# gopi-erabati/SRFDet3D

Hardware: AMD Instinct MI355X
Metric: frames/sec, srfdet_voxel_nusc_LC synthetic 30k-pt sweeps (higher is better)
Workload: dtype f32

## Files before the change

srfdet3d_amd/csrc/wino43.hip:

```cpp
#include "common.hpp"
#include <algorithm>

typedef float w43_f32x16 __attribute__((ext_vector_type(16)));
typedef float w43_f32x4 __attribute__((ext_vector_type(4)));
typedef float w43_v2 __attribute__((ext_vector_type(2)));

#define W43_TB 32
#define W43_PIECE 1024
#define W43_X1_BYTES (36 * 8 * 64 * 4)
#define W43_X_BYTES (36 * 16 * 64 * 4)

struct W43Args {
    const float *x;
    float *y;
    float *V;
    const float *U;
    const float *scale, *shift;
    long long x_ld, y_ld;
    int N, H, W, Cout;
    int tilesX, tilesY;
    long long ntiles;
    int ntb, nchunk, ncb, relu;
    int tb0, n0;
};

__global__ __launch_bounds__(256) void srf_wino43_pack_k(const float *__restrict__ Wt, int Cout, int Cin, int nchunk, float *__restrict__ P,
                                                        long long total)
{
    const long long t = (long long)blockIdx.x * 256 + threadIdx.x;
    if (t >= total) return;
    const int kk = (int)(t & 3), co = (int)((t >> 2) & 31), q = (int)((t >> 7) & 1), h = (int)((t >> 8) & 1);
    long long rest = t >> 9;
    const int f = (int)(rest % 36);
    rest /= 36;
    const int chunk = (int)(rest % nchunk), cb = (int)(rest / nchunk);
    const int cog = cb * 64 + h * 32 + co, ci = chunk * 8 + q * 4 + kk;
    float r = 0.f;
    if (cog < Cout) {
        const double G[6][3] = {{0.25, 0.0, 0.0},
                                {-1.0 / 6, -1.0 / 6, -1.0 / 6},
                                {-1.0 / 6, 1.0 / 6, -1.0 / 6},
                                {1.0 / 24, 1.0 / 12, 1.0 / 6},
                                {1.0 / 24, -1.0 / 12, 1.0 / 6},
                                {0.0, 0.0, 1.0}};
        const float *g = Wt + ((size_t)cog * Cin + ci) * 9;
        const int fr = f / 6, fs = f - fr * 6;
        double s = 0.0;
#pragma unroll
        for (int a = 0; a < 3; ++a)
#pragma unroll
            for (int b = 0; b < 3; ++b) s += G[fr][a] * (double)g[a * 3 + b] * G[fs][b];
        r = (float)s;
    }
    P[t] = r;
}

__device__ __forceinline__ float4 w43_fma4(float s, float4 a, float4 b)
{
    return make_float4(__fmaf_rn(s, a.x, b.x), __fmaf_rn(s, a.y, b.y), __fmaf_rn(s, a.z, b.z), __fmaf_rn(s, a.w, b.w));
}
__device__ __forceinline__ float4 w43_add4(float4 a, float4 b) { return make_float4(a.x + b.x, a.y + b.y, a.z + b.z, a.w + b.w); }
__device__ __forceinline__ float4 w43_sub4(float4 a, float4 b) { return make_float4(a.x - b.x, a.y - b.y, a.z - b.z, a.w - b.w); }

#define W43_BT(X0, X1, X2, X3, X4, X5, V0, V1, V2, V3, V4, V5)   \
    do {                                                         \
        const float4 a_ = w43_fma4(-4.f, X2, X4);                \
        const float4 b_ = w43_fma4(-4.f, X1, X3);                \
        const float4 c_ = w43_sub4(X4, X2);                      \
        const float4 e_ = w43_sub4(X3, X1);                      \
        const float4 v0_ = w43_fma4(4.f, X0, w43_fma4(-5.f, X2, X4)); \
        const float4 v5_ = w43_fma4(4.f, X1, w43_fma4(-5.f, X3, X5)); \
        V0 = v0_;                                                \
        V1 = w43_add4(a_, b_);                                   \
        V2 = w43_sub4(a_, b_);                                   \
        V3 = w43_fma4(2.f, e_, c_);                              \
        V4 = w43_fma4(-2.f, e_, c_);                             \
        V5 = v5_;                                                \
    } while (0)

__global__ __launch_bounds__(256) void srf_wino43_xform_k(W43Args a)
{
    const int tid = threadIdx.x, lane = tid & 63, wave = __builtin_amdgcn_readfirstlane(tid >> 6);
    const int cgroups = (a.nchunk + 3) >> 2;
    const int tbl = blockIdx.x / cgroups, cg = blockIdx.x - tbl * cgroups;
    const int qd = lane & 7, t = wave * 8 + (lane >> 3);
    const int c = cg * 4 + (qd >> 1), q = qd & 1;
    const bool c_ok = c < a.nchunk;
    const int g = (a.tb0 + tbl) * W43_TB + t;
    const int per_img = a.tilesX * a.tilesY;
    const bool live = g < (int)a.ntiles;
    const int n = live ? g / per_img : a.n0;
    const int rem = live ? g - n * per_img : 0;
    const int ty = rem / a.tilesX, tx = rem - ty * a.tilesX;
    const long long img_b = (long long)a.H * a.W * a.x_ld * 4;
    const long long left_b = (long long)(a.N - a.n0) * img_b;
    __amdgpu_buffer_rsrc_t xr = __builtin_amdgcn_make_buffer_rsrc(const_cast<float *>(a.x), 0,
                                                                 (int)(unsigned)(left_b < 0xFFFFFFF0ll ? left_b : 0xFFFFFFF0ll), 0x00020000);
    const int y0 = 4 * ty - 1, x0 = 4 * tx - 1;
    const unsigned px_b = (unsigned)(a.x_ld * 4);
    const unsigned chan_b = (unsigned)((c * 8 + q * 4) * 4) + (unsigned)(n - a.n0) * (unsigned)img_b;
    const bool share = (lane < 56) && live && (g + 1 < (int)a.ntiles) && (tx + 1 < a.tilesX);
    float4 d[6][6];
#pragma unroll
    for (int py = 0; py < 6; ++py) {
        const int y = y0 + py;
        const bool yok = live && c_ok && y >= 0 && y < a.H;
        const unsigned row_b = (unsigned)(y * a.W) * px_b + chan_b;
#pragma unroll
        for (int px = 0; px < 6; ++px) {
            const int x = x0 + px;
            const bool ok = yok && x >= 0 && x < a.W && !(px >= 4 && share);
            const unsigned off = ok ? row_b + (unsigned)x * px_b : 0xFFFFFFF8u;
            auto v_ = __builtin_amdgcn_raw_buffer_load_b128(xr, (int)off, 0, 0);
            d[py][px] = *reinterpret_cast<float4 *>(&v_);
        }
    }
#pragma unroll
    for (int py = 0; py < 6; ++py)
#pragma unroll
        for (int px = 4; px < 6; ++px) {
            const float4 nb = d[py][px - 4];
            const float sx = __shfl_down(nb.x, 8), sy = __shfl_down(nb.y, 8), sz = __shfl_down(nb.z, 8), sw = __shfl_down(nb.w, 8);
            if (share) d[py][px] = make_float4(sx, sy, sz, sw);
        }
    if (!c_ok) return;
#pragma unroll
    for (int px = 0; px < 6; ++px)
        W43_BT(d[0][px], d[1][px], d[2][px], d[3][px], d[4][px], d[5][px], d[0][px], d[1][px], d[2][px], d[3][px], d[4][px], d[5][px]);
    float4 *vp = reinterpret_cast<float4 *>(a.V) + ((size_t)tbl * a.nchunk + c) * (36 * 64) + q * 32 + t;
#pragma unroll
    for (int r = 0; r < 6; ++r) {
        float4 v0, v1, v2, v3, v4, v5;
        W43_BT(d[r][0], d[r][1], d[r][2], d[r][3], d[r][4], d[r][5], v0, v1, v2, v3, v4, v5);
        vp[(r * 6 + 0) * 64] = v0;
        vp[(r * 6 + 1) * 64] = v1;
        vp[(r * 6 + 2) * 64] = v2;
        vp[(r * 6 + 3) * 64] = v3;
        vp[(r * 6 + 4) * 64] = v4;
        vp[(r * 6 + 5) * 64] = v5;
    }
}

__device__ __forceinline__ w43_v2 w43_pk_add(w43_v2 a, w43_v2 b)
{
    w43_v2 r;
    asm("v_pk_add_f32 %0, %1, %2" : "=v"(r) : "v"(a), "v"(b));
    return r;
}
__device__ __forceinline__ w43_v2 w43_pk_sub(w43_v2 a, w43_v2 b)
{
    w43_v2 r;
    asm("v_pk_add_f32 %0, %1, %2 neg_lo:[0,1] neg_hi:[0,1]" : "=v"(r) : "v"(a), "v"(b));
    return r;
}
__device__ __forceinline__ w43_v2 w43_pk_fma(w43_v2 s, w43_v2 a, w43_v2 b)
{
    w43_v2 r;
    asm("v_pk_fma_f32 %0, %1, %2, %3" : "=v"(r) : "v"(s), "v"(a), "v"(b));
    return r;
}
#define W43_AT(M0, M1, M2, M3, M4, M5, Z0, Z1, Z2, Z3)           \
    do {                                                         \
        const w43_v2 s1_ = w43_pk_add(M1, M2), d1_ = w43_pk_sub(M1, M2); \
        const w43_v2 s2_ = w43_pk_add(M3, M4), d2_ = w43_pk_sub(M3, M4); \
        Z0 = w43_pk_add(w43_pk_add(M0, s1_), s2_);               \
        Z1 = w43_pk_fma(k2_, d2_, d1_);                          \
        Z2 = w43_pk_fma(k4_, s2_, s1_);                          \
        Z3 = w43_pk_add(w43_pk_fma(k8_, d2_, d1_), M5);          \
    } while (0)

#define W43_MFMA(ACC, A, B) ACC = __builtin_amdgcn_mfma_f32_32x32x2f32(A, B, ACC, 0, 0, 0)

template <int NB>
__device__ __forceinline__ void srf_wino43_mm_body(const W43Args &a, const int tb, const int hb)
{
    extern __shared__ __attribute__((aligned(16))) float s_x[];
    const int tid = threadIdx.x, lane = tid & 63, wave = __builtin_amdgcn_readfirstlane(tid >> 6);
    const int li = lane & 31, lh = lane >> 5;
    const int cb = hb >> 1, h0 = hb & 1;
    const int nchunk = a.nchunk;
    __amdgpu_buffer_rsrc_t vr = __builtin_amdgcn_make_buffer_rsrc(
        const_cast<float *>(a.V) + (size_t)(tb - a.tb0) * nchunk * (36 * 256), 0, (int)((long long)nchunk * 36 * W43_PIECE), 0x00020000);
    __amdgpu_buffer_rsrc_t ur = __builtin_amdgcn_make_buffer_rsrc(
        const_cast<float *>(a.U) + (size_t)cb * nchunk * (36 * 2 * 256), 0, (int)((long long)nchunk * 36 * 2 * W43_PIECE), 0x00020000);
    const int voff = lane * 16;
    const int fbase = wave * 9;

    w43_f32x16 acc[9][NB];
    w43_f32x4 fa[9], fb[9][NB];
#define W43_LOAD(J, C)                                                                                                   \
    do {                                                                                                                 \
        const int sa_ = ((C) * 36 + fbase + (J)) * W43_PIECE;                                                            \
        auto va_ = __builtin_amdgcn_raw_buffer_load_b128(vr, voff, sa_, 0);                                              \
        fa[J] = *reinterpret_cast<w43_f32x4 *>(&va_);                                                                    \
        _Pragma("unroll") for (int h_ = 0; h_ < NB; ++h_) {                                                              \
            const int sb_ = (((C) * 36 + fbase + (J)) * 2 + (NB == 2 ? h_ : h0)) * W43_PIECE;                            \
            auto vb_ = __builtin_amdgcn_raw_buffer_load_b128(ur, voff, sb_, 0);                                          \
            fb[J][h_] = *reinterpret_cast<w43_f32x4 *>(&vb_);                                                            \
        }                                                                                                                \
    } while (0)
#define W43_MFMA_V(ACC, A, B) asm volatile("v_mfma_f32_32x32x2_f32 %0, %1, %2, %0" : "+v"(ACC) : "v"(A), "v"(B))
#define W43_MFMA_V0(ACC, A, B) asm volatile("v_mfma_f32_32x32x2_f32 %0, %1, %2, 0" : "=&v"(ACC) : "v"(A), "v"(B))
#define W43_GROUP(J, FIRST)                                                                                              \
    do {                                                                                                                 \
        _Pragma("unroll") for (int s_ = 0; s_ < 4; ++s_)                                                                 \
            _Pragma("unroll") for (int h_ = 0; h_ < NB; ++h_) {                                                          \
                if (NB == 2 && (J) == 8) {                                                                               \
                    if ((FIRST) && s_ == 0) W43_MFMA_V0(acc[J][h_], fa[J][s_], fb[J][h_][s_]);                           \
                    else W43_MFMA_V(acc[J][h_], fa[J][s_], fb[J][h_][s_]);                                               \
                } else if ((FIRST) && s_ == 0) {                                                                         \
                    const w43_f32x16 z_ = {0.f, 0.f, 0.f, 0.f, 0.f, 0.f, 0.f, 0.f, 0.f, 0.f, 0.f, 0.f, 0.f, 0.f, 0.f, 0.f}; \
                    acc[J][h_] = __builtin_amdgcn_mfma_f32_32x32x2f32(fa[J][s_], fb[J][h_][s_], z_, 0, 0, 0);            \
                } else                                                                                                   \
                    W43_MFMA(acc[J][h_], fa[J][s_], fb[J][h_][s_]);                                                      \
            }                                                                                                            \
    } while (0)

#pragma unroll
    for (int j = 0; j < 9; ++j) W43_LOAD(j, 0);
    if (nchunk > 1) {
#pragma unroll
        for (int j = 0; j < 9; ++j) {
            W43_GROUP(j, 1);
            W43_LOAD(j, 1);
            __builtin_amdgcn_sched_barrier(0);
        }
        for (int c = 1; c < nchunk - 1; ++c) {
#pragma unroll
            for (int j = 0; j < 9; ++j) {
                W43_GROUP(j, 0);
                W43_LOAD(j, c + 1);
                __builtin_amdgcn_sched_barrier(0);
            }
        }
#pragma unroll
        for (int j = 0; j < 9; ++j) W43_GROUP(j, 0);
    } else {
#pragma unroll
        for (int j = 0; j < 9; ++j) W43_GROUP(j, 1);
    }

    asm volatile("s_nop 15\n\ts_nop 15" ::: "memory");
    const w43_v2 k2_ = {2.f, 2.f}, k4_ = {4.f, 4.f}, k8_ = {8.f, 8.f};
    float *X = s_x;
    const int per_img = a.tilesX * a.tilesY;
    const unsigned ypx_b = (unsigned)(a.y_ld * 4), yrow_b = (unsigned)a.W * ypx_b;
    const long long yleft_b = (long long)(a.N - a.n0) * a.H * a.W * a.y_ld * 4;
    __amdgpu_buffer_rsrc_t yr = __builtin_amdgcn_make_buffer_rsrc(a.y, 0, (int)(unsigned)(yleft_b < 0xFFFFFFF0ll ? yleft_b : 0xFFFFFFF0ll), 0x00020000);
    if constexpr (NB == 1) {
        const w43_v2 *X2 = reinterpret_cast<const w43_v2 *>(s_x);
        const int er = tid >> 5, ep = tid & 31;
        const int co = cb * 64 + h0 * 32 + 2 * (ep & 15);
        const bool co_ok = co < a.Cout;
        w43_v2 sc = {1.f, 1.f}, sh = {0.f, 0.f};
        if (co_ok && a.scale) sc = *reinterpret_cast<const w43_v2 *>(a.scale + co);
        if (co_ok && a.shift) sh = *reinterpret_cast<const w43_v2 *>(a.shift + co);
#pragma unroll
        for (int ph = 0; ph < 2; ++ph) {
            const int r = ph * 8 + er;
            const int et = (r & 3) + 8 * (r >> 2) + 4 * (ep >> 4);
            const int eg = tb * W43_TB + et;
            const bool elive = eg < (int)a.ntiles;
            const int en = elive ? eg / per_img : a.n0;
            const int erem = elive ? eg - en * per_img : 0;
            const int ety = erem / a.tilesX, etx = erem - ety * a.tilesX;
            const int rows_ok = elive ? min(4, a.H - 4 * ety) : 0, cols_ok = min(4, a.W - 4 * etx);
            const unsigned ebase = (unsigned)(en - a.n0) * ((unsigned)a.H * yrow_b) + (unsigned)(4 * ety) * yrow_b + (unsigned)(4 * etx) * ypx_b;
            __syncthreads();
#pragma unroll
            for (int j = 0; j < 9; ++j)
#pragma unroll
                for (int rr = 0; rr < 8; ++rr) X[((fbase + j) * 8 + rr) * 64 + lane] = acc[j][0][ph * 8 + rr];
            __syncthreads();
            w43_v2 z[4][6];
#pragma unroll
            for (int s = 0; s < 6; ++s) {
                const w43_v2 m0 = X2[((0 * 6 + s) * 8 + er) * 32 + ep], m1 = X2[((1 * 6 + s) * 8 + er) * 32 + ep],
                             m2 = X2[((2 * 6 + s) * 8 + er) * 32 + ep], m3 = X2[((3 * 6 + s) * 8 + er) * 32 + ep],
                             m4 = X2[((4 * 6 + s) * 8 + er) * 32 + ep], m5 = X2[((5 * 6 + s) * 8 + er) * 32 + ep];
                W43_AT(m0, m1, m2, m3, m4, m5, z[0][s], z[1][s], z[2][s], z[3][s]);
            }
#pragma unroll
            for (int i = 0; i < 4; ++i) {
                w43_v2 o[4];
                W43_AT(z[i][0], z[i][1], z[i][2], z[i][3], z[i][4], z[i][5], o[0], o[1], o[2], o[3]);
#pragma unroll
                for (int jx = 0; jx < 4; ++jx) {
                    w43_v2 v = w43_pk_fma(o[jx], sc, sh);
                    if (a.relu) {
                        v[0] = fmaxf(v[0], 0.f);
                        v[1] = fmaxf(v[1], 0.f);
                    }
                    const bool ok = co_ok && i < rows_ok && jx < cols_ok;
                    const unsigned off = ok ? ebase + (unsigned)i * yrow_b + (unsigned)jx * ypx_b + (unsigned)co * 4u : 0xFFFFFFF8u;
                    typedef unsigned w43_u2 __attribute__((ext_vector_type(2)));
                    const w43_u2 bits = {__float_as_uint(v[0]), __float_as_uint(v[1])};
                    __builtin_amdgcn_raw_buffer_store_b64(bits, yr, (int)off, 0, 0);
                }
            }
        }
    } else {
    const float4 *X4 = reinterpret_cast<const float4 *>(s_x);
    const int er = tid >> 4, eq = tid & 15;
    const int et = (er & 3) + 8 * (er >> 2) + 4 * (eq >> 3);
    const int co4 = (eq & 7) * 4;
    const int eg = tb * W43_TB + et;
    const bool elive = eg < (int)a.ntiles;
    const int en = elive ? eg / per_img : a.n0;
    const int erem = elive ? eg - en * per_img : 0;
    const int ety = erem / a.tilesX, etx = erem - ety * a.tilesX;
    const int rows_ok = elive ? min(4, a.H - 4 * ety) : 0, cols_ok = min(4, a.W - 4 * etx);
    const unsigned ebase = (unsigned)(en - a.n0) * ((unsigned)a.H * yrow_b) + (unsigned)(4 * ety) * yrow_b + (unsigned)(4 * etx) * ypx_b;
#pragma unroll
    for (int p = 0; p < NB; ++p) {
        __syncthreads();
#pragma unroll
        for (int j = 0; j < 9; ++j)
#pragma unroll
            for (int r = 0; r < 16; ++r) X[((fbase + j) * 16 + r) * 64 + lane] = acc[j][p][r];
        __syncthreads();
        const int co = cb * 64 + (NB == 2 ? p : h0) * 32 + co4;
        const bool co_ok = co < a.Cout;
        float4 sc = make_float4(1.f, 1.f, 1.f, 1.f), sh = make_float4(0.f, 0.f, 0.f, 0.f);
        if (co_ok && a.scale) sc = *reinterpret_cast<const float4 *>(a.scale + co);
        if (co_ok && a.shift) sh = *reinterpret_cast<const float4 *>(a.shift + co);
        const w43_v2 scl = {sc.x, sc.y}, sch = {sc.z, sc.w}, shl = {sh.x, sh.y}, shh = {sh.z, sh.w};
        w43_v2 zl[4][6], zh[4][6];
#pragma unroll
        for (int s = 0; s < 6; ++s) {
            float4 m[6];
#pragma unroll
            for (int r = 0; r < 6; ++r) m[r] = X4[((r * 6 + s) * 16 + er) * 16 + eq];
            const w43_v2 l0 = {m[0].x, m[0].y}, l1 = {m[1].x, m[1].y}, l2 = {m[2].x, m[2].y}, l3 = {m[3].x, m[3].y}, l4 = {m[4].x, m[4].y},
                         l5 = {m[5].x, m[5].y};
            const w43_v2 h0_ = {m[0].z, m[0].w}, h1 = {m[1].z, m[1].w}, h2 = {m[2].z, m[2].w}, h3 = {m[3].z, m[3].w}, h4 = {m[4].z, m[4].w},
                         h5 = {m[5].z, m[5].w};
            W43_AT(l0, l1, l2, l3, l4, l5, zl[0][s], zl[1][s], zl[2][s], zl[3][s]);
            W43_AT(h0_, h1, h2, h3, h4, h5, zh[0][s], zh[1][s], zh[2][s], zh[3][s]);
        }
#pragma unroll
        for (int i = 0; i < 4; ++i) {
            w43_v2 ol[4], oh[4];
            W43_AT(zl[i][0], zl[i][1], zl[i][2], zl[i][3], zl[i][4], zl[i][5], ol[0], ol[1], ol[2], ol[3]);
            W43_AT(zh[i][0], zh[i][1], zh[i][2], zh[i][3], zh[i][4], zh[i][5], oh[0], oh[1], oh[2], oh[3]);
#pragma unroll
            for (int jx = 0; jx < 4; ++jx) {
                w43_v2 vl = w43_pk_fma(ol[jx], scl, shl), vh = w43_pk_fma(oh[jx], sch, shh);
                if (a.relu) {
                    vl[0] = fmaxf(vl[0], 0.f);
                    vl[1] = fmaxf(vl[1], 0.f);
                    vh[0] = fmaxf(vh[0], 0.f);
                    vh[1] = fmaxf(vh[1], 0.f);
                }
                const bool ok = co_ok && i < rows_ok && jx < cols_ok;
                const unsigned off = ok ? ebase + (unsigned)i * yrow_b + (unsigned)jx * ypx_b + (unsigned)co * 4u : 0xFFFFFFF8u;
                typedef unsigned w43_u4 __attribute__((ext_vector_type(4)));
                const w43_u4 bits = {__float_as_uint(vl[0]), __float_as_uint(vl[1]), __float_as_uint(vh[0]), __float_as_uint(vh[1])};
                __builtin_amdgcn_raw_buffer_store_b128(bits, yr, (int)off, 0, 0);
            }
        }
    }
    }
}

template <int NB>
__global__ __launch_bounds__(256, NB == 1 ? 2 : 1) void srf_wino43_mm_k(W43Args a, int nitems_cb)
{
    const int xcd = blockIdx.x & 7, jq = blockIdx.x >> 3;
    const int cbi = jq % nitems_cb;
    const int tb = a.tb0 + (jq / nitems_cb) * 8 + xcd;
    if (tb >= a.ntb) return;
    srf_wino43_mm_body<NB>(a, tb, NB == 2 ? 2 * cbi : cbi);
}

extern "C" size_t srf_wino43_packed_weight_bytes(int Cout, int Cin)
{
    if (Cout <= 0 || Cin <= 0 || (Cin & 7)) return 0;
    return (size_t)srf_ceil_div(Cout, 64) * (Cin / 8) * 36 * 2 * W43_PIECE;
}

extern "C" int srf_wino43_pack_weights(const float *W, int Cout, int Cin, float *packed, srf_stream_t stream)
{
    if (Cout <= 0 || Cin <= 0 || !W || !packed) return SRF_EINVAL;
    if (Cin & 7) return SRF_EUNSUPPORTED;
    const long long total = (long long)(srf_wino43_packed_weight_bytes(Cout, Cin) / 4);
    hipLaunchKernelGGL(srf_wino43_pack_k, dim3((unsigned)srf_ceil_div(total, 256)), dim3(256), 0, (hipStream_t)stream, W, Cout, Cin, Cin / 8,
                       packed, total);
    SRF_LAUNCH_CHECK();
    return SRF_OK;
}

#define W43_SLAB_BYTES (2048ll << 20)

static long long w43_slab_tb(long long ntb, int nchunk, int ncb)
{
    static const long long forced = srf_knob("SRF_W43_SLAB_TB", 0);
    if (forced > 0) return forced < ntb ? forced : ntb;
    const long long per_tb = (long long)nchunk * 36 * W43_PIECE;
    long long fit = W43_SLAB_BYTES / per_tb;
    if (fit < 8) fit = 8;
    if (fit >= ntb) return ntb;
    const long long round = (256 + ncb - 1) / ncb;
    long long k = fit / round;
    if (k < 1) k = 1;
    long long slab = k * round;
    slab = (slab + 7) / 8 * 8;
    return slab < ntb ? slab : ntb;
}

extern "C" size_t srf_wino43_workspace_bytes(int N, int H, int W, int Cin, int Cout)
{
    if (N <= 0 || H <= 0 || W <= 0 || Cin <= 0 || Cout <= 0 || (Cin & 7)) return 0;
    const long long ntiles = (long long)N * srf_ceil_div(H, 4) * srf_ceil_div(W, 4);
    const long long ntb = (ntiles + W43_TB - 1) / W43_TB;
    return (size_t)w43_slab_tb(ntb, Cin / 8, srf_ceil_div(Cout, 64)) * (Cin / 8) * 36 * W43_PIECE;
}

#define W43_NEED_X 1
#define W43_NEED_Y 2
static int w43_make_args(W43Args &a, const float *x, int N, int H, int W, int Cin, long long x_ld, const float *U_packed, int Cout,
                         const float *scale, const float *shift, int relu, float *y, long long y_ld, void *workspace, size_t workspace_bytes,
                         int need = W43_NEED_X | W43_NEED_Y)
{
    if (N < 0 || H <= 0 || W <= 0 || Cin <= 0 || Cout <= 0) return SRF_EINVAL;
    if (((need & W43_NEED_X) && x_ld < Cin) || ((need & W43_NEED_Y) && y_ld < Cout)) return SRF_EINVAL;
    if (N == 0) return SRF_OK;
    if (!workspace || ((need & W43_NEED_X) && !x) || ((need & W43_NEED_Y) && (!U_packed || !y))) return SRF_EINVAL;
    if ((Cin & 7) || (Cout & 3) || ((uintptr_t)workspace & 15)) return SRF_EUNSUPPORTED;
    if ((need & W43_NEED_X) && ((x_ld & 3) || ((uintptr_t)x & 15))) return SRF_EUNSUPPORTED;
    if ((need & W43_NEED_Y) && ((y_ld & 3) || ((uintptr_t)y & 15) || ((uintptr_t)U_packed & 15) || (scale && ((uintptr_t)scale & 15)) ||
                                (shift && ((uintptr_t)shift & 15))))
        return SRF_EUNSUPPORTED;
    if (workspace_bytes < srf_wino43_workspace_bytes(N, H, W, Cin, Cout)) return SRF_EWORKSPACE;
    a.x = x;
    a.y = y;
    a.V = (float *)workspace;
    a.U = U_packed;
    a.scale = scale;
    a.shift = shift;
    a.x_ld = x_ld;
    a.y_ld = y_ld;
    a.N = N;
    a.H = H;
    a.W = W;
    a.Cout = Cout;
    a.tilesX = srf_ceil_div(W, 4);
    a.tilesY = srf_ceil_div(H, 4);
    a.ntiles = (long long)N * a.tilesX * a.tilesY;
    const long long ntb = (a.ntiles + W43_TB - 1) / W43_TB;
    a.nchunk = Cin / 8;
    a.ncb = srf_ceil_div(Cout, 64);
    a.relu = relu;
    a.tb0 = 0;
    a.n0 = 0;
    if (a.ntiles + W43_TB >= (1ll << 31) || ntb * ((a.nchunk + 3) / 4) >= (1ll << 31) || ntb * a.ncb * 2 >= (1ll << 30)) return SRF_EUNSUPPORTED;
    if ((long long)a.nchunk * 36 * 2 * W43_PIECE >= (1ll << 31)) return SRF_EUNSUPPORTED;
    a.ntb = (int)ntb;
    return SRF_OK;
}

static int w43_slab_args(const W43Args &full, long long tb0, long long cnt, W43Args &s)
{
    s = full;
    const long long per_img = (long long)full.tilesX * full.tilesY;
    const long long g0 = tb0 * W43_TB, g1 = std::min((tb0 + cnt) * W43_TB, full.ntiles) - 1;
    const long long n0 = g0 / per_img, n1 = g1 / per_img;
    const long long ximg = (long long)full.H * full.W * full.x_ld * 4, yimg = (long long)full.H * full.W * full.y_ld * 4;
    if ((n1 - n0 + 1) * ximg >= 0xFFFFFFF0ll || (n1 - n0 + 1) * yimg >= 0xFFFFFFF0ll) return SRF_EUNSUPPORTED;
    s.tb0 = (int)tb0;
    s.ntb = (int)(tb0 + cnt);
    s.n0 = (int)n0;
    s.x = full.x + n0 * (ximg / 4);
    s.y = full.y + n0 * (yimg / 4);
    return SRF_OK;
}

static int w43_launch_xform(const W43Args &a, hipStream_t stream)
{
    hipLaunchKernelGGL(srf_wino43_xform_k, dim3((unsigned)((long long)(a.ntb - a.tb0) * ((a.nchunk + 3) / 4))), dim3(256), 0, stream, a);
    SRF_LAUNCH_CHECK();
    return SRF_OK;
}

static int w43_launch_mm(const W43Args &a, hipStream_t stream)
{
    int dev = 0;
    SRF_HIP_TRY(hipGetDevice(&dev));
    if (dev < 0 || dev >= 64) return SRF_EUNSUPPORTED;
    static bool attr_set[64] = {false};
    if (!attr_set[dev]) {
        SRF_HIP_TRY(hipFuncSetAttribute((const void *)srf_wino43_mm_k<2>, hipFuncAttributeMaxDynamicSharedMemorySize, W43_X_BYTES));
        SRF_HIP_TRY(hipFuncSetAttribute((const void *)srf_wino43_mm_k<1>, hipFuncAttributeMaxDynamicSharedMemorySize, W43_X1_BYTES));
        attr_set[dev] = true;
    }
    const long long tb8 = (((long long)(a.ntb - a.tb0) + 7) / 8) * 8;
    static const int force_nb = srf_knob("SRF_W43_NB", 0);
    const int nb = force_nb ? (force_nb == 1 ? 1 : 2) : (((a.Cout & 63) == 0 && (long long)(a.ntb - a.tb0) * a.ncb >= 1024) ? 2 : 1);
    if (nb == 1) {
        const int nhb = srf_ceil_div(a.Cout, 32);
        hipLaunchKernelGGL((srf_wino43_mm_k<1>), dim3((unsigned)(tb8 * nhb)), dim3(256), W43_X1_BYTES, stream, a, nhb);
    } else
        hipLaunchKernelGGL((srf_wino43_mm_k<2>), dim3((unsigned)(tb8 * a.ncb)), dim3(256), W43_X_BYTES, stream, a, a.ncb);
    SRF_LAUNCH_CHECK();
    return SRF_OK;
}

extern "C" int srf_wino43(const float *x, int N, int H, int W, int Cin, long long x_ld, const float *U_packed, int Cout, const float *scale,
                          const float *shift, int relu, float *y, long long y_ld, void *workspace, size_t workspace_bytes, srf_stream_t stream)
{
    W43Args a;
    const int rc = w43_make_args(a, x, N, H, W, Cin, x_ld, U_packed, Cout, scale, shift, relu, y, y_ld, workspace, workspace_bytes);
    if (rc != SRF_OK || N == 0) return rc;
    const long long slab = w43_slab_tb(a.ntb, a.nchunk, a.ncb);
    for (long long tb0 = 0; tb0 < a.ntb; tb0 += slab) {
        W43Args s;
        const int r0 = w43_slab_args(a, tb0, std::min(slab, (long long)a.ntb - tb0), s);
        if (r0 != SRF_OK) return r0;
    }
    for (long long tb0 = 0; tb0 < a.ntb; tb0 += slab) {
        W43Args s;
        w43_slab_args(a, tb0, std::min(slab, (long long)a.ntb - tb0), s);
        const int r1 = w43_launch_xform(s, (hipStream_t)stream);
        if (r1 != SRF_OK) return r1;
        const int r2 = w43_launch_mm(s, (hipStream_t)stream);
        if (r2 != SRF_OK) return r2;
    }
    return SRF_OK;
}

extern "C" int srf_wino43_transform(const float *x, int N, int H, int W, int Cin, long long x_ld, int Cout, void *workspace,
                                    size_t workspace_bytes, srf_stream_t stream)
{
    W43Args a;
    const int rc = w43_make_args(a, x, N, H, W, Cin, x_ld, nullptr, Cout, nullptr, nullptr, 0, nullptr, 4, workspace, workspace_bytes, W43_NEED_X);
    if (rc != SRF_OK || N == 0) return rc;
    if (w43_slab_tb(a.ntb, a.nchunk, a.ncb) < a.ntb) return SRF_EUNSUPPORTED;
    W43Args s;
    const int r0 = w43_slab_args(a, 0, a.ntb, s);
    if (r0 != SRF_OK) return r0;
    return w43_launch_xform(s, (hipStream_t)stream);
}

extern "C" int srf_wino43_multiply(const void *workspace, size_t workspace_bytes, int N, int H, int W, int Cin, const float *U_packed,
                                   int Cout, const float *scale, const float *shift, int relu, float *y, long long y_ld, srf_stream_t stream)
{
    W43Args a;
    const int rc = w43_make_args(a, nullptr, N, H, W, Cin, 4, U_packed, Cout, scale, shift, relu, y, y_ld, const_cast<void *>(workspace),
                                 workspace_bytes, W43_NEED_Y);
    if (rc != SRF_OK || N == 0) return rc;
    if (w43_slab_tb(a.ntb, a.nchunk, a.ncb) < a.ntb) return SRF_EUNSUPPORTED;
    W43Args s;
    const int r0 = w43_slab_args(a, 0, a.ntb, s);
    if (r0 != SRF_OK) return r0;
    return w43_launch_mm(s, (hipStream_t)stream);
}
```

srfdet3d_amd/csrc/gemm_split.hip:

```cpp
#include "common.hpp"
#include "gemm_tile128.hpp"

typedef __bf16 gs_bf2 __attribute__((ext_vector_type(2)));
typedef __bf16 gs_bf8 __attribute__((ext_vector_type(8)));
typedef float gs_f2 __attribute__((ext_vector_type(2)));
typedef float gs_f4 __attribute__((ext_vector_type(4)));
typedef float gs_f16 __attribute__((ext_vector_type(16)));
typedef unsigned gs_u2 __attribute__((ext_vector_type(2)));
typedef unsigned gs_u4 __attribute__((ext_vector_type(4)));

#define GS_IMG 24576

struct GsArgs : SrfTile128Args<const unsigned char *> {
    int H, W, Ho, Wo, kw, stride, pad, cin_chunks;
    long long x_bytes;
};
#define GS_PLAIN 0
#define GS_POOL 1
#define GS_TOPDOWN 2
#define GS_CONV 3
#define GS_RESID 4

__device__ __forceinline__ unsigned gs_pk_bf16(float a, float b)
{
    const gs_f2 v = {a, b};
    const gs_bf2 h = __builtin_convertvector(v, gs_bf2);
    return *reinterpret_cast<const unsigned *>(&h);
}

__device__ __forceinline__ void gs_split2(float x0, float x1, unsigned &h, unsigned &m, unsigned &l)
{
    h = gs_pk_bf16(x0, x1);
    const float r0 = __fsub_rn(x0, __uint_as_float(h << 16)), r1 = __fsub_rn(x1, __uint_as_float(h & 0xffff0000u));
    m = gs_pk_bf16(r0, r1);
    const float s0 = __fsub_rn(r0, __uint_as_float(m << 16)), s1 = __fsub_rn(r1, __uint_as_float(m & 0xffff0000u));
    l = gs_pk_bf16(s0, s1);
}

__global__ __launch_bounds__(256) void srf_gemm_split_pack_k(const float *__restrict__ Wt, int Cout, int K, int nct, unsigned short *__restrict__ P,
                                                            long long total)
{
    const long long t = (long long)blockIdx.x * 256 + threadIdx.x;
    if (t >= total) return;
    const int e = (int)(t & 7), s = (int)((t >> 3) & 3), n = (int)((t >> 5) & 127);
    long long rest = t >> 12;
    const int p = (int)(rest % 3);
    rest /= 3;
    const int ct = (int)(rest % nct), c = (int)(rest / nct);
    const int oct = s ^ ((n >> 2) & 3);
    const int k = c * 32 + oct * 8 + e, co = ct * 128 + n;
    const float x = co < Cout ? Wt[(size_t)co * K + k] : 0.f;
    unsigned h, m, l;
    gs_split2(x, 0.f, h, m, l);
    P[t] = (unsigned short)((p == 0 ? h : p == 1 ? m : l) & 0xffffu);
}

template <int MODE>
__global__ __launch_bounds__(256, MODE == GS_CONV ? 2 : 3) void srf_gemm_split_k(GsArgs a)
{
    constexpr bool POOL = MODE == GS_POOL, TOPDOWN = MODE == GS_TOPDOWN, CONV = MODE == GS_CONV, RESID = MODE == GS_RESID;
    __shared__ __attribute__((aligned(16))) unsigned char lds[2 * GS_IMG];
    const int tid = threadIdx.x, lane = tid & 63, wave = __builtin_amdgcn_readfirstlane(tid >> 6);
    int ct;
    const long long mb = srf_tile128_row_block(a.nct, ct);
    if (mb >= a.mblocks) return;
    const SrfTile128Item it = srf_tile128_item<POOL>(ct, mb, a.M, a.HW, a.bpi);
    const long long p0 = it.p0, rows_here = it.rows_here;
    __amdgpu_buffer_rsrc_t xr = CONV ? __builtin_amdgcn_make_buffer_rsrc(const_cast<float *>(a.x), 0, (int)a.x_bytes, 0x00020000)
                                     : __builtin_amdgcn_make_buffer_rsrc(const_cast<float *>(a.x) + p0 * a.x_ld, 0, (int)(rows_here * a.x_ld * 4), 0x00020000);
    const int nchunk = a.nchunk;
    const size_t chunk_stride = (size_t)a.nct * GS_IMG;
    const unsigned char *bsrc = a.Wp + (size_t)ct * GS_IMG + (size_t)tid * 16;

    const int q = tid & 7, r0 = tid >> 3;
    const unsigned aoff0 = (unsigned)((r0 * a.x_ld + q * 4) * 4), aoff_step = (unsigned)(32 * a.x_ld * 4);
    gs_f4 araw[4];
    gs_u4 braw[6];
    unsigned sp[3][4][2];
    int cy[CONV ? 4 : 1], cx[CONV ? 4 : 1], cn[CONV ? 4 : 1];
    if (CONV) {
#pragma unroll
        for (int j = 0; j < 4; ++j) {
            const long long p = p0 + r0 + 32 * j;
            const long long hw = (long long)a.Ho * a.Wo;
            const int n = (int)(p / hw);
            const int rem = (int)(p - n * hw);
            const int oy = rem / a.Wo, ox = rem - oy * a.Wo;
            cn[j] = p < a.M ? n : -1;
            cy[j] = oy * a.stride - a.pad;
            cx[j] = ox * a.stride - a.pad;
        }
    }
#define GS_LOAD(C)                                                                                                         \
    do {                                                                                                                   \
        if (CONV) {                                                                                                        \
            const int tap_ = (C) / a.cin_chunks, cc_ = (C) - tap_ * a.cin_chunks;                                          \
            const int ky_ = tap_ / a.kw, kx_ = tap_ - ky_ * a.kw;                                                          \
            _Pragma("unroll") for (int j_ = 0; j_ < 4; ++j_) {                                                             \
                const int iy_ = cy[j_] + ky_, ix_ = cx[j_] + kx_;                                                          \
                const bool ok_ = cn[j_] >= 0 && iy_ >= 0 && iy_ < a.H && ix_ >= 0 && ix_ < a.W;                            \
                const unsigned off_ = ok_ ? (unsigned)(((((long long)cn[j_] * a.H + iy_) * a.W + ix_) * a.x_ld + cc_ * 32 + q * 4) * 4) \
                                          : 0x80000000u;                                                                   \
                auto v_ = __builtin_amdgcn_raw_buffer_load_b128(xr, (int)off_, 0, 0);                                      \
                araw[j_] = *reinterpret_cast<gs_f4 *>(&v_);                                                                \
            }                                                                                                              \
        } else {                                                                                                           \
            _Pragma("unroll") for (int j_ = 0; j_ < 4; ++j_) {                                                             \
                auto v_ = __builtin_amdgcn_raw_buffer_load_b128(xr, (int)(aoff0 + j_ * aoff_step), (C) * 128, 0);          \
                araw[j_] = *reinterpret_cast<gs_f4 *>(&v_);                                                                \
            }                                                                                                              \
        }                                                                                                                  \
        const gs_u4 *bb_ = reinterpret_cast<const gs_u4 *>(bsrc + (size_t)(C) * chunk_stride);                             \
        _Pragma("unroll") for (int i_ = 0; i_ < 6; ++i_) braw[i_] = bb_[i_ * 256];                                         \
    } while (0)
#define GS_SPLIT()                                                                                                         \
    do {                                                                                                                   \
        _Pragma("unroll") for (int j_ = 0; j_ < 4; ++j_) {                                                                 \
            gs_split2(araw[j_][0], araw[j_][1], sp[0][j_][0], sp[1][j_][0], sp[2][j_][0]);                                 \
            gs_split2(araw[j_][2], araw[j_][3], sp[0][j_][1], sp[1][j_][1], sp[2][j_][1]);                                 \
        }                                                                                                                  \
    } while (0)
#define GS_STORE()                                                                                                         \
    do {                                                                                                                   \
        _Pragma("unroll") for (int j_ = 0; j_ < 4; ++j_) {                                                                 \
            const int row_ = r0 + 32 * j_;                                                                                 \
            const int off_ = row_ * 64 + (((q >> 1) ^ ((row_ >> 2) & 3)) << 4) + (q & 1) * 8;                              \
            _Pragma("unroll") for (int p_ = 0; p_ < 3; ++p_) {                                                             \
                const gs_u2 w_ = {sp[p_][j_][0], sp[p_][j_][1]};                                                           \
                *reinterpret_cast<gs_u2 *>(lds + p_ * 8192 + off_) = w_;                                                   \
            }                                                                                                              \
        }                                                                                                                  \
        _Pragma("unroll") for (int i_ = 0; i_ < 6; ++i_) *reinterpret_cast<gs_u4 *>(lds + GS_IMG + (tid + i_ * 256) * 16) = braw[i_]; \
    } while (0)

    const int wm = wave & 1, wn = wave >> 1;
    const int li = lane & 31, lh = lane >> 5;
    int a_off[2], b_off[2], swz_a[2], swz_b[2];
#pragma unroll
    for (int i = 0; i < 2; ++i) {
        const int row = wm * 64 + i * 32 + li, col = wn * 64 + i * 32 + li;
        a_off[i] = row * 64;
        b_off[i] = GS_IMG + col * 64;
        swz_a[i] = (row >> 2) & 3;
        swz_b[i] = (col >> 2) & 3;
    }
    gs_f16 acc[2][2];
#pragma unroll
    for (int i = 0; i < 2; ++i)
#pragma unroll
        for (int j = 0; j < 2; ++j)
#pragma unroll
            for (int r = 0; r < 16; ++r) acc[i][j][r] = 0.f;
    gs_bf8 fa[3][2], fb[3][2];
#define GS_READ(S)                                                                                                         \
    do {                                                                                                                   \
        _Pragma("unroll") for (int p_ = 0; p_ < 3; ++p_)                                                                   \
            _Pragma("unroll") for (int i_ = 0; i_ < 2; ++i_) {                                                             \
                fa[p_][i_] = *reinterpret_cast<const gs_bf8 *>(lds + p_ * 8192 + a_off[i_] + (((2 * (S) + lh) ^ swz_a[i_]) << 4)); \
                fb[p_][i_] = *reinterpret_cast<const gs_bf8 *>(lds + p_ * 8192 + b_off[i_] + (((2 * (S) + lh) ^ swz_b[i_]) << 4)); \
            }                                                                                                              \
    } while (0)
#define GS_MM(PA, PB)                                                                                                      \
    _Pragma("unroll") for (int i_ = 0; i_ < 2; ++i_)                                                                       \
        _Pragma("unroll") for (int j_ = 0; j_ < 2; ++j_)                                                                   \
            acc[i_][j_] = __builtin_amdgcn_mfma_f32_32x32x16_bf16(fa[PA][i_], fb[PB][j_], acc[i_][j_], 0, 0, 0)
#define GS_MFMA6() do { GS_MM(2, 0); GS_MM(0, 2); GS_MM(1, 1); GS_MM(1, 0); GS_MM(0, 1); GS_MM(0, 0); } while (0)

    const int last = nchunk - 1;
    GS_LOAD(0);
    GS_SPLIT();
    GS_STORE();
    GS_LOAD(last < 1 ? last : 1);
    __syncthreads();
    for (int c = 0; c < nchunk; ++c) {
        const int c2 = c + 2 < nchunk ? c + 2 : last;
        GS_READ(0);
        GS_MFMA6();
        GS_SPLIT();
        GS_READ(1);
        GS_MFMA6();
        __syncthreads();
        GS_STORE();
        GS_LOAD(c2);
        __syncthreads();
    }
#undef GS_LOAD
#undef GS_SPLIT
#undef GS_STORE
#undef GS_READ
#undef GS_MM
#undef GS_MFMA6

    srf_tile128_epilogue<POOL, TOPDOWN, RESID>(SRF_TILE128_EPI(a), acc, it, lds, tid, li, lh, wm, wn);
}

extern "C" size_t srf_conv1x1_nhwc_split_packed_weight_bytes(int Cout, int K)
{
    if (Cout <= 0 || K <= 0 || (K & 31)) return 0;
    return (size_t)(K / 32) * srf_ceil_div(Cout, 128) * GS_IMG;
}

extern "C" int srf_conv1x1_nhwc_split_pack_weights(const float *W, int Cout, int K, void *packed, srf_stream_t stream)
{
    if (Cout <= 0 || K <= 0 || !W || !packed) return SRF_EINVAL;
    if (K & 31) return SRF_EUNSUPPORTED;
    const int nct = srf_ceil_div(Cout, 128);
    const long long total = (long long)(srf_conv1x1_nhwc_split_packed_weight_bytes(Cout, K) / 2);
    hipLaunchKernelGGL(srf_gemm_split_pack_k, dim3((unsigned)srf_ceil_div(total, 256)), dim3(256), 0, (hipStream_t)stream, W, Cout, K, nct,
                       (unsigned short *)packed, total);
    SRF_LAUNCH_CHECK();
    return SRF_OK;
}

struct GsFamily {
    typedef GsArgs Args;
    static constexpr SrfGemmFamily limits = {128, true, 128};
    static constexpr void (*plain)(GsArgs) = srf_gemm_split_k<GS_PLAIN>, (*pool)(GsArgs) = srf_gemm_split_k<GS_POOL>,
                          (*topdown)(GsArgs) = srf_gemm_split_k<GS_TOPDOWN>, (*resid)(GsArgs) = srf_gemm_split_k<GS_RESID>,
                          (*conv)(GsArgs) = srf_gemm_split_k<GS_CONV>;
    static int set_weights(GsArgs &a, const void *W_packed)
    {
        a.Wp = (const unsigned char *)W_packed;
        return SRF_OK;
    }
};

extern "C" int srf_conv_gemm_nhwc_split(const float *x, int N, int H, int W, int Cin, long long x_ld, const void *W_packed, int Cout, int kh,
                                        int kw, int stride, int pad, const float *scale, const float *shift, int relu, float *y,
                                        long long y_ld, srf_stream_t stream)
{
    return srf_tile128_conv<GsFamily>(x, N, H, W, Cin, x_ld, W_packed, Cout, kh, kw, stride, pad, scale, shift, relu, y, y_ld, stream);
}

extern "C" int srf_conv1x1_nhwc_split(const float *x, long long M, int K, long long x_ld, const void *W_packed, int Cout, const float *scale,
                                      const float *shift, int relu, float *y, long long y_ld, srf_stream_t stream)
{
    return srf_tile128_plain<GsFamily>(x, M, K, x_ld, W_packed, Cout, scale, shift, relu, y, y_ld, stream);
}

extern "C" int srf_conv1x1_nhwc_split_residual(const float *x, long long M, int K, long long x_ld, const void *W_packed, int Cout, const float *scale,
                                               const float *shift, int relu, float *y, long long y_ld, const float *res, long long res_ld,
                                               srf_stream_t stream)
{
    return srf_tile128_residual<GsFamily>(x, M, K, x_ld, W_packed, Cout, scale, shift, relu, y, y_ld, res, res_ld, stream);
}

extern "C" int srf_conv1x1_nhwc_split_topdown(const float *x, int N, int H, int W, int K, long long x_ld, const void *W_packed, int Cout,
                                              const float *scale, const float *shift, int relu, const float *top, int Ht, int Wt,
                                              long long top_ld, float *y, long long y_ld, srf_stream_t stream)
{
    return srf_tile128_topdown<GsFamily>(x, N, H, W, K, x_ld, W_packed, Cout, scale, shift, relu, top, Ht, Wt, top_ld, y, y_ld, stream);
}

extern "C" int srf_conv1x1_nhwc_split_pooled(const float *x, int N, long long HW, int K, long long x_ld, const void *W_packed, int Cout,
                                             const float *scale, const float *shift, int relu, float *y, long long y_ld, float *mean,
                                             void *workspace, size_t workspace_bytes, srf_stream_t stream)
{
    return srf_tile128_pooled<GsFamily>(x, N, HW, K, x_ld, W_packed, Cout, scale, shift, relu, y, y_ld, mean, workspace, workspace_bytes, stream);
}
```

Before: 30.44.

## Add Winograd input-transform variants with half-width lanes and XCD-aware block swizzle

Templates the Winograd F(4,3) input-transform kernel on vector width (float4 or float2 per lane) and on how many waves share a tile group versus spread over channel chunks. An optional block-index swizzle puts consecutive tile blocks on the same XCD. A heuristic picks one of three forms from the tile-block count and channel chunks. The aim is more blocks and better cache locality when the grid is small, at the cost of more shuffle and load instructions per byte in the float2 form and of blocks that exit early when the swizzled grid is padded.

```diff
diff --git a/srfdet3d_amd/csrc/wino43.hip b/srfdet3d_amd/csrc/wino43.hip
--- a/srfdet3d_amd/csrc/wino43.hip
+++ b/srfdet3d_amd/csrc/wino43.hip
@@ -61,15 +61,18 @@
 }
 __device__ __forceinline__ float4 w43_add4(float4 a, float4 b) { return make_float4(a.x + b.x, a.y + b.y, a.z + b.z, a.w + b.w); }
 __device__ __forceinline__ float4 w43_sub4(float4 a, float4 b) { return make_float4(a.x - b.x, a.y - b.y, a.z - b.z, a.w - b.w); }
+__device__ __forceinline__ float2 w43_fma4(float s, float2 a, float2 b) { return make_float2(__fmaf_rn(s, a.x, b.x), __fmaf_rn(s, a.y, b.y)); }
+__device__ __forceinline__ float2 w43_add4(float2 a, float2 b) { return make_float2(a.x + b.x, a.y + b.y); }
+__device__ __forceinline__ float2 w43_sub4(float2 a, float2 b) { return make_float2(a.x - b.x, a.y - b.y); }
 
 #define W43_BT(X0, X1, X2, X3, X4, X5, V0, V1, V2, V3, V4, V5)   \
     do {                                                         \
-        const float4 a_ = w43_fma4(-4.f, X2, X4);                \
-        const float4 b_ = w43_fma4(-4.f, X1, X3);                \
-        const float4 c_ = w43_sub4(X4, X2);                      \
-        const float4 e_ = w43_sub4(X3, X1);                      \
-        const float4 v0_ = w43_fma4(4.f, X0, w43_fma4(-5.f, X2, X4)); \
-        const float4 v5_ = w43_fma4(4.f, X1, w43_fma4(-5.f, X3, X5)); \
+        const auto a_ = w43_fma4(-4.f, X2, X4);                  \
+        const auto b_ = w43_fma4(-4.f, X1, X3);                  \
+        const auto c_ = w43_sub4(X4, X2);                        \
+        const auto e_ = w43_sub4(X3, X1);                        \
+        const auto v0_ = w43_fma4(4.f, X0, w43_fma4(-5.f, X2, X4)); \
+        const auto v5_ = w43_fma4(4.f, X1, w43_fma4(-5.f, X3, X5)); \
         V0 = v0_;                                                \
         V1 = w43_add4(a_, b_);                                   \
         V2 = w43_sub4(a_, b_);                                   \
@@ -78,13 +81,54 @@
         V5 = v5_;                                                \
     } while (0)
 
-__global__ __launch_bounds__(256) void srf_wino43_xform_k(W43Args a)
-{
+template <int VEC>
+struct w43_lane;
+template <>
+struct w43_lane<4> {
+    typedef float4 T;
+    static __device__ __forceinline__ T load(__amdgpu_buffer_rsrc_t r, unsigned off)
+    {
+        auto v_ = __builtin_amdgcn_raw_buffer_load_b128(r, (int)off, 0, 0);
+        return *reinterpret_cast<T *>(&v_);
+    }
+    static __device__ __forceinline__ T down8(T v) { return make_float4(__shfl_down(v.x, 8), __shfl_down(v.y, 8), __shfl_down(v.z, 8), __shfl_down(v.w, 8)); }
+};
+template <>
+struct w43_lane<2> {
+    typedef float2 T;
+    static __device__ __forceinline__ T load(__amdgpu_buffer_rsrc_t r, unsigned off)
+    {
+        auto v_ = __builtin_amdgcn_raw_buffer_load_b64(r, (int)off, 0, 0);
+        return *reinterpret_cast<T *>(&v_);
+    }
+    static __device__ __forceinline__ T down8(T v) { return make_float2(__shfl_down(v.x, 8), __shfl_down(v.y, 8)); }
+};
+
+template <int VEC, int TW>
+__global__ __launch_bounds__(256) void srf_wino43_xform_k(W43Args a, int swz)
+{
+    typedef w43_lane<VEC> L;
+    typedef typename L::T VT;
+    constexpr int CW = 4 / TW;
     const int tid = threadIdx.x, lane = tid & 63, wave = __builtin_amdgcn_readfirstlane(tid >> 6);
-    const int cgroups = (a.nchunk + 3) >> 2;
-    const int tbl = blockIdx.x / cgroups, cg = blockIdx.x - tbl * cgroups;
-    const int qd = lane & 7, t = wave * 8 + (lane >> 3);
-    const int c = cg * 4 + (qd >> 1), q = qd & 1;
+    const int csg = (a.nchunk + VEC * CW - 1) / (VEC * CW);
+    const int per_tb = CW * csg;
+    int tbl, within;
+    if (swz) {
+        const int xcd = blockIdx.x & 7, jq = blockIdx.x >> 3;
+        tbl = (jq / per_tb) * 8 + xcd;
+        within = jq % per_tb;
+        if (tbl >= a.ntb - a.tb0) return;
+    } else {
+        tbl = blockIdx.x / per_tb;
+        within = blockIdx.x - tbl * per_tb;
+    }
+    const int og = within / csg, cs = within - og * csg;
+    const int wt = wave / CW, wc = wave - wt * CW;
+    const int slice = cs * CW + wc;
+    if (slice * VEC >= a.nchunk) return;
+    const int qd = lane & 7, t = (og * TW + wt) * 8 + (lane >> 3);
+    const int c = slice * VEC + (VEC == 4 ? (qd >> 1) : (qd >> 2)), q = VEC == 4 ? (qd & 1) : ((qd >> 1) & 1), h = VEC == 4 ? 0 : (qd & 1);
     const bool c_ok = c < a.nchunk;
     const int g = (a.tb0 + tbl) * W43_TB + t;
     const int per_img = a.tilesX * a.tilesY;
@@ -98,9 +142,9 @@
                                                                  (int)(unsigned)(left_b < 0xFFFFFFF0ll ? left_b : 0xFFFFFFF0ll), 0x00020000);
     const int y0 = 4 * ty - 1, x0 = 4 * tx - 1;
     const unsigned px_b = (unsigned)(a.x_ld * 4);
-    const unsigned chan_b = (unsigned)((c * 8 + q * 4) * 4) + (unsigned)(n - a.n0) * (unsigned)img_b;
+    const unsigned chan_b = (unsigned)((c * 8 + q * 4 + h * 2) * 4) + (unsigned)(n - a.n0) * (unsigned)img_b;
     const bool share = (lane < 56) && live && (g + 1 < (int)a.ntiles) && (tx + 1 < a.tilesX);
-    float4 d[6][6];
+    VT d[6][6];
 #pragma unroll
     for (int py = 0; py < 6; ++py) {
         const int y = y0 + py;
@@ -111,33 +155,31 @@
             const int x = x0 + px;
             const bool ok = yok && x >= 0 && x < a.W && !(px >= 4 && share);
             const unsigned off = ok ? row_b + (unsigned)x * px_b : 0xFFFFFFF8u;
-            auto v_ = __builtin_amdgcn_raw_buffer_load_b128(xr, (int)off, 0, 0);
-            d[py][px] = *reinterpret_cast<float4 *>(&v_);
+            d[py][px] = L::load(xr, off);
         }
     }
 #pragma unroll
     for (int py = 0; py < 6; ++py)
 #pragma unroll
         for (int px = 4; px < 6; ++px) {
-            const float4 nb = d[py][px - 4];
-            const float sx = __shfl_down(nb.x, 8), sy = __shfl_down(nb.y, 8), sz = __shfl_down(nb.z, 8), sw = __shfl_down(nb.w, 8);
-            if (share) d[py][px] = make_float4(sx, sy, sz, sw);
+            const VT nb = L::down8(d[py][px - 4]);
+            if (share) d[py][px] = nb;
         }
     if (!c_ok) return;
 #pragma unroll
     for (int px = 0; px < 6; ++px)
         W43_BT(d[0][px], d[1][px], d[2][px], d[3][px], d[4][px], d[5][px], d[0][px], d[1][px], d[2][px], d[3][px], d[4][px], d[5][px]);
-    float4 *vp = reinterpret_cast<float4 *>(a.V) + ((size_t)tbl * a.nchunk + c) * (36 * 64) + q * 32 + t;
+    float *vf = a.V + (((size_t)tbl * a.nchunk + c) * (36 * 64) + q * 32 + t) * 4 + h * 2;
 #pragma unroll
     for (int r = 0; r < 6; ++r) {
-        float4 v0, v1, v2, v3, v4, v5;
+        VT v0, v1, v2, v3, v4, v5;
         W43_BT(d[r][0], d[r][1], d[r][2], d[r][3], d[r][4], d[r][5], v0, v1, v2, v3, v4, v5);
-        vp[(r * 6 + 0) * 64] = v0;
-        vp[(r * 6 + 1) * 64] = v1;
-        vp[(r * 6 + 2) * 64] = v2;
-        vp[(r * 6 + 3) * 64] = v3;
-        vp[(r * 6 + 4) * 64] = v4;
-        vp[(r * 6 + 5) * 64] = v5;
+        *reinterpret_cast<VT *>(vf + (r * 6 + 0) * 256) = v0;
+        *reinterpret_cast<VT *>(vf + (r * 6 + 1) * 256) = v1;
+        *reinterpret_cast<VT *>(vf + (r * 6 + 2) * 256) = v2;
+        *reinterpret_cast<VT *>(vf + (r * 6 + 3) * 256) = v3;
+        *reinterpret_cast<VT *>(vf + (r * 6 + 4) * 256) = v4;
+        *reinterpret_cast<VT *>(vf + (r * 6 + 5) * 256) = v5;
     }
 }
 
@@ -475,11 +517,38 @@
     return SRF_OK;
 }
 
-static int w43_launch_xform(const W43Args &a, hipStream_t stream)
-{
-    hipLaunchKernelGGL(srf_wino43_xform_k, dim3((unsigned)((long long)(a.ntb - a.tb0) * ((a.nchunk + 3) / 4))), dim3(256), 0, stream, a);
+#define W43_XF_FORMS 3
+template <int VEC, int TW>
+static int w43_launch_xform_as(const W43Args &a, int swz, hipStream_t stream)
+{
+    const long long ntbl = a.ntb - a.tb0, per_tb = (4 / TW) * (long long)((a.nchunk + VEC * (4 / TW) - 1) / (VEC * (4 / TW)));
+    const long long grid = (swz ? (ntbl + 7) / 8 * 8 : ntbl) * per_tb;
+    if (grid >= (1ll << 31)) return SRF_EUNSUPPORTED;
+    hipLaunchKernelGGL((srf_wino43_xform_k<VEC, TW>), dim3((unsigned)grid), dim3(256), 0, stream, a, swz);
     SRF_LAUNCH_CHECK();
     return SRF_OK;
+}
+
+static int w43_launch_xform_form(const W43Args &a, int form, hipStream_t stream)
+{
+    switch (form) {
+    case 1: return w43_launch_xform_as<4, 4>(a, 0, stream);
+    case 2: return w43_launch_xform_as<4, 2>(a, 1, stream);
+    case 3: return w43_launch_xform_as<2, 1>(a, 1, stream);
+    }
+    return SRF_EINVAL;
+}
+
+static int w43_xform_form(long long ntbl, int nchunk)
+{
+    if (ntbl < 64) return 1;
+    return ntbl * ((nchunk + 3) / 4) <= 320 ? 3 : 2;
+}
+
+static int w43_launch_xform(const W43Args &a, hipStream_t stream)
+{
+    static const int forced = (int)srf_knob("SRF_W43_XF", 0);
+    return w43_launch_xform_form(a, forced > 0 ? forced : w43_xform_form(a.ntb - a.tb0, a.nchunk), stream);
 }
 
 static int w43_launch_mm(const W43Args &a, hipStream_t stream)
```

New measurement: 30.47, median of 2. About the same (+0.1%).

## Stream split-GEMM weight tiles directly into LDS via buffer_load lds DMA

Applied to the files above, without the earlier changes.

Replaces the register-staged global-to-LDS copy of packed B weight tiles with inline-asm buffer_load_dwordx4 ... lds instructions that write straight into shared memory through M0. The main loop is restructured: the second half-step's LDS fragments are read into a separate register set before the barrier, so the next chunk's store, DMA and A-load can be issued while the second group of MFMAs runs. __syncthreads is replaced by custom waitcnt+barrier macros, one of which waits only for vmcnt(4). This aims to free VGPRs and overlap weight traffic with compute, at the cost of fragile hand-written waitcnt and M0 handling and extra fragment registers.

```diff
diff --git a/srfdet3d_amd/csrc/gemm_split.hip b/srfdet3d_amd/csrc/gemm_split.hip
--- a/srfdet3d_amd/csrc/gemm_split.hip
+++ b/srfdet3d_amd/csrc/gemm_split.hip
@@ -35,6 +35,35 @@
     m = gs_pk_bf16(r0, r1);
     const float s0 = __fsub_rn(r0, __uint_as_float(m << 16)), s1 = __fsub_rn(r1, __uint_as_float(m & 0xffff0000u));
     l = gs_pk_bf16(s0, s1);
+}
+
+__device__ __forceinline__ void gs_dma_b(gs_u4 desc, unsigned voff, unsigned lds_dst)
+{
+    unsigned keep;
+    asm volatile("s_nop 4\n\t"
+                 "s_mov_b32 %0, m0\n\t"
+                 "s_mov_b32 m0, %3\n\t"
+                 "s_nop 0\n\t"
+                 "buffer_load_dwordx4 %1, %2, 0 offen lds\n\t"
+                 "s_add_u32 m0, m0, 0x1000\n\t"
+                 "s_nop 0\n\t"
+                 "buffer_load_dwordx4 %1, %2, %4 offen lds\n\t"
+                 "s_add_u32 m0, m0, 0x1000\n\t"
+                 "s_nop 0\n\t"
+                 "buffer_load_dwordx4 %1, %2, %5 offen lds\n\t"
+                 "s_add_u32 m0, m0, 0x1000\n\t"
+                 "s_nop 0\n\t"
+                 "buffer_load_dwordx4 %1, %2, %6 offen lds\n\t"
+                 "s_add_u32 m0, m0, 0x1000\n\t"
+                 "s_nop 0\n\t"
+                 "buffer_load_dwordx4 %1, %2, %7 offen lds\n\t"
+                 "s_add_u32 m0, m0, 0x1000\n\t"
+                 "s_nop 0\n\t"
+                 "buffer_load_dwordx4 %1, %2, %8 offen lds\n\t"
+                 "s_mov_b32 m0, %0"
+                 : "=&s"(keep)
+                 : "v"(voff), "s"(desc), "s"(lds_dst), "s"(4096), "s"(8192), "s"(12288), "s"(16384), "s"(20480)
+                 : "memory", "scc");
 }
 
 __global__ __launch_bounds__(256) void srf_gemm_split_pack_k(const float *__restrict__ Wt, int Cout, int K, int nct, unsigned short *__restrict__ P,
@@ -70,12 +99,13 @@
                                      : __builtin_amdgcn_make_buffer_rsrc(const_cast<float *>(a.x) + p0 * a.x_ld, 0, (int)(rows_here * a.x_ld * 4), 0x00020000);
     const int nchunk = a.nchunk;
     const size_t chunk_stride = (size_t)a.nct * GS_IMG;
-    const unsigned char *bsrc = a.Wp + (size_t)ct * GS_IMG + (size_t)tid * 16;
+    const unsigned char *bbase = a.Wp + (size_t)ct * GS_IMG;
+    const unsigned lds_bw = (unsigned)(size_t)(__attribute__((address_space(3))) unsigned char *)lds + GS_IMG + (unsigned)wave * 1024u;
+    const unsigned bvoff = (unsigned)tid * 16u;
 
     const int q = tid & 7, r0 = tid >> 3;
     const unsigned aoff0 = (unsigned)((r0 * a.x_ld + q * 4) * 4), aoff_step = (unsigned)(32 * a.x_ld * 4);
     gs_f4 araw[4];
-    gs_u4 braw[6];
     unsigned sp[3][4][2];
     int cy[CONV ? 4 : 1], cx[CONV ? 4 : 1], cn[CONV ? 4 : 1];
     if (CONV) {
@@ -110,8 +140,12 @@
                 araw[j_] = *reinterpret_cast<gs_f4 *>(&v_);                                                                \
             }                                                                                                              \
         }                                                                                                                  \
-        const gs_u4 *bb_ = reinterpret_cast<const gs_u4 *>(bsrc + (size_t)(C) * chunk_stride);                             \
-        _Pragma("unroll") for (int i_ = 0; i_ < 6; ++i_) braw[i_] = bb_[i_ * 256];                                         \
+    } while (0)
+#define GS_DMA_B(C)                                                                                                        \
+    do {                                                                                                                   \
+        const unsigned long long g_ = (unsigned long long)(bbase + (size_t)(C) * chunk_stride);                            \
+        const gs_u4 d_ = {(unsigned)g_, (unsigned)(g_ >> 32), (unsigned)GS_IMG, 0x00020000u};                              \
+        gs_dma_b(d_, bvoff, lds_bw);                                                                                       \
     } while (0)
 #define GS_SPLIT()                                                                                                         \
     do {                                                                                                                   \
@@ -130,8 +164,10 @@
                 *reinterpret_cast<gs_u2 *>(lds + p_ * 8192 + off_) = w_;                                                   \
             }                                                                                                              \
         }                                                                                                                  \
-        _Pragma("unroll") for (int i_ = 0; i_ < 6; ++i_) *reinterpret_cast<gs_u4 *>(lds + GS_IMG + (tid + i_ * 256) * 16) = braw[i_]; \
     } while (0)
+#define GS_BAR_READS() asm volatile("s_waitcnt lgkmcnt(0)\n\ts_barrier" ::: "memory")
+#define GS_BAR_STAGED() asm volatile("s_waitcnt vmcnt(4) lgkmcnt(0)\n\ts_barrier" ::: "memory")
+#define GS_PIN_ACC() asm volatile("" : "+v"(acc[0][0]), "+v"(acc[0][1]), "+v"(acc[1][0]), "+v"(acc[1][1]))
 
     const int wm = wave & 1, wn = wave >> 1;
     const int li = lane & 31, lh = lane >> 5;
@@ -151,42 +187,49 @@
         for (int j = 0; j < 2; ++j)
 #pragma unroll
             for (int r = 0; r < 16; ++r) acc[i][j][r] = 0.f;
-    gs_bf8 fa[3][2], fb[3][2];
-#define GS_READ(S)                                                                                                         \
-    do {                                                                                                                   \
-        _Pragma("unroll") for (int p_ = 0; p_ < 3; ++p_)                                                                   \
-            _Pragma("unroll") for (int i_ = 0; i_ < 2; ++i_) {                                                             \
-                fa[p_][i_] = *reinterpret_cast<const gs_bf8 *>(lds + p_ * 8192 + a_off[i_] + (((2 * (S) + lh) ^ swz_a[i_]) << 4)); \
-                fb[p_][i_] = *reinterpret_cast<const gs_bf8 *>(lds + p_ * 8192 + b_off[i_] + (((2 * (S) + lh) ^ swz_b[i_]) << 4)); \
-            }                                                                                                              \
-    } while (0)
-#define GS_MM(PA, PB)                                                                                                      \
+    gs_bf8 fa[3][2], fb[3][2], ga[3][2], gb[3][2];
+#define GS_READ(FA, FB, S, P)                                                                                              \
+    _Pragma("unroll") for (int i_ = 0; i_ < 2; ++i_) {                                                                     \
+        FA[P][i_] = *reinterpret_cast<const gs_bf8 *>(lds + (P) * 8192 + a_off[i_] + (((2 * (S) + lh) ^ swz_a[i_]) << 4)); \
+        FB[P][i_] = *reinterpret_cast<const gs_bf8 *>(lds + (P) * 8192 + b_off[i_] + (((2 * (S) + lh) ^ swz_b[i_]) << 4)); \
+    }
+#define GS_MM(FA, FB, PA, PB)                                                                                              \
     _Pragma("unroll") for (int i_ = 0; i_ < 2; ++i_)                                                                       \
         _Pragma("unroll") for (int j_ = 0; j_ < 2; ++j_)                                                                   \
-            acc[i_][j_] = __builtin_amdgcn_mfma_f32_32x32x16_bf16(fa[PA][i_], fb[PB][j_], acc[i_][j_], 0, 0, 0)
-#define GS_MFMA6() do { GS_MM(2, 0); GS_MM(0, 2); GS_MM(1, 1); GS_MM(1, 0); GS_MM(0, 1); GS_MM(0, 0); } while (0)
+            acc[i_][j_] = __builtin_amdgcn_mfma_f32_32x32x16_bf16(FA[PA][i_], FB[PB][j_], acc[i_][j_], 0, 0, 0)
+#define GS_MFMA6(FA, FB)                                                                                                   \
+    do { GS_MM(FA, FB, 2, 0); GS_MM(FA, FB, 0, 2); GS_MM(FA, FB, 1, 1); GS_MM(FA, FB, 1, 0); GS_MM(FA, FB, 0, 1); GS_MM(FA, FB, 0, 0); } while (0)
 
     const int last = nchunk - 1;
     GS_LOAD(0);
     GS_SPLIT();
     GS_STORE();
+    GS_DMA_B(0);
     GS_LOAD(last < 1 ? last : 1);
-    __syncthreads();
+    GS_BAR_STAGED();
     for (int c = 0; c < nchunk; ++c) {
         const int c2 = c + 2 < nchunk ? c + 2 : last;
-        GS_READ(0);
-        GS_MFMA6();
+        GS_READ(fa, fb, 0, 2) GS_READ(fa, fb, 0, 0) GS_READ(fa, fb, 0, 1)
+        GS_MFMA6(fa, fb);
         GS_SPLIT();
-        GS_READ(1);
-        GS_MFMA6();
-        __syncthreads();
+        GS_PIN_ACC();
+        __builtin_amdgcn_sched_barrier(0);
+        GS_READ(ga, gb, 1, 2) GS_READ(ga, gb, 1, 1) GS_READ(ga, gb, 1, 0)
+        GS_BAR_READS();
         GS_STORE();
+        if (c < last) GS_DMA_B(c + 1);
         GS_LOAD(c2);
-        __syncthreads();
+        GS_MFMA6(ga, gb);
+        GS_PIN_ACC();
+        GS_BAR_STAGED();
     }
 #undef GS_LOAD
+#undef GS_DMA_B
 #undef GS_SPLIT
 #undef GS_STORE
+#undef GS_BAR_READS
+#undef GS_BAR_STAGED
+#undef GS_PIN_ACC
 #undef GS_READ
 #undef GS_MM
 #undef GS_MFMA6
```

New measurement: 30.69 before, 30.60 after. About the same (-0.3%).
